# PatrizioPerugini/depth_completion_MT

Hardware: AMD Instinct MI355X
Metric: depth frames/sec at 1216x352 (KITTI); achieved HBM GB/s vs peak (higher is better)
Workload: dtype f32

## Files before the change

### depth_completion_mt_amd/csrc/dcmt.hip

```cpp
#include <hip/hip_runtime.h>

#include <cmath>
#include <cstdio>
#include <cstdlib>
#include <cstdint>
#include <cstring>
#include <algorithm>
#include <new>
#include <type_traits>
#include <vector>

#include "dcmt.h"
#include "dcmt_plan.h"
#include "dcmt_kernels_v1.h"
#include "dcmt_kernels_fused.h"
#include "dcmt_kernels_pair.h"
#include "dcmt_kernels_fp_q16.h"
#include "dcmt_kernels_tail.h"
#include "dcmt_kernels_slic.h"
#include "dcmt_kernels_eval.h"
#include "dcmt_kernels_color.h"
#include "dcmt_cloud.h"

using namespace dcmt;
// ... 47 lines not shown
    uint32_t* cloud_slab = nullptr;
};

namespace {

using plan::TH;
using plan::TW;
using plan::FTH_FEW;

static_assert(plan::kK0AsCompiled == K0_AS_COMPILED && plan::kK0Diamond == K0_DIAMOND, "k0 presets");
static_assert(plan::pre_p_vw(K0_AS_COMPILED, false) == PreP<K0_AS_COMPILED, false>::VW && plan::pre_p_vw(K0_DIAMOND, false) == PreP<K0_DIAMOND, false>::VW &&
              plan::pre_p_vw(K0_AS_COMPILED, true) == PreP<K0_AS_COMPILED, true>::VW && plan::pre_p_vw(K0_DIAMOND, true) == PreP<K0_DIAMOND, true>::VW, "PreP::VW");
static_assert(plan::pre_s_vw(K0_AS_COMPILED, false) == PreS<K0_AS_COMPILED, false>::VW && plan::pre_s_vw(K0_AS_COMPILED, true) == PreS<K0_AS_COMPILED, true>::VW &&
              plan::pre_s_vw(K0_DIAMOND, false) == PreS<K0_DIAMOND, false>::VW && plan::pre_s_vw(K0_DIAMOND, true) == PreS<K0_DIAMOND, true>::VW, "PreS::VW");
static_assert(plan::kFpQVW == FpQ::VW && plan::kPostSVW == PostS::VW && plan::kFillSVW == FillS::VW, "FpQ / PostS / FillS::VW");
static_assert(plan::kMaxBands == kMaxBands && plan::kLabelGroupMax == kLabelGroupMax, "kMaxBands, kLabelGroupMax");
static_assert(plan::kStageNormalize == DCMT_STAGE_NORMALIZE && plan::kStageClose5 == DCMT_STAGE_CLOSE5 && plan::kStageFill7 == DCMT_STAGE_FILL7 &&
              plan::kStageExtend == DCMT_STAGE_EXTEND && plan::kStageFinal == DCMT_STAGE_FINAL, "dcmt_stage");
static_assert(plan::kFlagForceStaged == DCMT_FLAG_FORCE_STAGED && plan::kFlagForceFused == DCMT_FLAG_FORCE_FUSED &&
              plan::kFlagNormalize == DCMT_FLAG_NORMALIZE, "DCMT_FLAG_*");
static_assert(plan::q16_params_ok(100.0f, 0.1f) && Q16::params_ok(100.0f, 0.1f) && !plan::q16_params_ok(80.0f, 0.1f) && !Q16::params_ok(80.0f, 0.1f) &&
              !plan::q16_params_ok(100.0f, 0.2f) && !Q16::params_ok(100.0f, 0.2f), "Q16::params_ok");
static_assert(sizeof(plan::Plan::path) == sizeof(dcmt_ctx::last_path), "dcmt_last_path");

#define DCMT_HIP(ctx, call)                                        \
    do {                                                           \
        hipError_t e_ = (call);                                    \
        if (e_ != hipSuccess) {                                    \
            if (ctx) (ctx)->last_hip_error = (int)e_;              \
            return e_ == hipErrorOutOfMemory ? DCMT_E_NOMEM : DCMT_E_HIP; \
// ... 194 lines not shown
    const float scale = src16 ? fr.in_scale : 1.0f;
    auto pre_s = [&](auto kind, auto wide_) {
        constexpr int KIND = decltype(kind)::value;
        constexpr bool WIDE = decltype(wide_)::value;
        auto* k = d_x4 ? k_pre_s<KIND, WIDE, true, false> : src16 ? k_pre_s<KIND, false, false, true> :
                  cf ? k_pre_s<KIND, WIDE, false, false, true> : k_pre_s<KIND, WIDE, false, false>;
        hipLaunchKernelGGL(k, dim3(pl.pre_grid), b256, 0, st, in, o6, rows, cols, pl.pre_strips, batch, xm, p->max_depth, p->valid_thresh,
                           scale, cf, tc, cnt);
    };
    auto pre_p = [&](auto kind, auto qout, float* o, int* qbad, const int* gate, int* qclr) {
        constexpr int KIND = decltype(kind)::value;
        constexpr bool QOUT = decltype(qout)::value;
        auto* k = d_x4 ? k_pre_p<KIND, true, false, false, QOUT> : src16 ? k_pre_p<KIND, false, true, false, QOUT> :
                  cf ? k_pre_p<KIND, false, false, true> : k_pre_p<KIND, false, false, false, QOUT>;
        hipLaunchKernelGGL(k, dim3(pl.pre_grid), b256, 0, st, in, o, rows, cols, pl.pre_strips, bands, batch, xm, p->max_depth,
                           p->valid_thresh, scale, cf, tc, cnt, qbad, gate, ctx->q16_seen_dev, qclr);
    };
    int* qbad = ctx->q16_bad;
    if (q16) {
        qbad = ctx->q16_bad + ctx->q16_attempts % kQ16Flags;
        int* qnext = ctx->q16_bad + (ctx->q16_attempts + 1) % kQ16Flags;
        ++ctx->q16_attempts;
        with_k0(pl.k0kind, [&](auto kind) { pre_p(kind, std::true_type{}, reinterpret_cast<float*>(ctx->x6q), qbad, nullptr, qnext); });
    } else if (pl.pair) {
        with_k0(pl.k0kind, [&](auto kind) { pre_p(kind, std::false_type{}, o6, nullptr, nullptr, nullptr); });
    } else {
        with_k0(pl.k0kind, [&](auto kind) { if (pl.wide) pre_s(kind, std::true_type{}); else pre_s(kind, std::false_type{}); });
    }
    DCMT_HIP(ctx, hipGetLastError());
    stamp(2);
    if (stop == DCMT_STAGE_EXTEND) {
// ... 2 lines not shown
    }

    const int fstrips = pl.fill_strips, pstrips = pl.post_strips;
    const dim3 fgrid(pl.fill_grid);
    auto fill_apps = [&](int* apps) {
        return fill_loop(ctx, batch, p, st, sync_loop, [&](int i) {
            hipLaunchKernelGGL(k_fill_s, fgrid, b256, 0, st, (i & 1) ? pp0 : pp1, (i & 1) ? pp1 : pp0, cnt, rows, cols,
                               fstrips, batch, xm, p->valid_thresh, i, 0, (const int*)nullptr, 1, (const unsigned short*)nullptr, (const int*)nullptr);
        }, apps);
    };
    if (pl.fuse_fp) {
        const int n_redo = pl.n_redo;
        if (q16) {
            auto* fpq = filled ? k_fp_q<true, true> : bl ? k_fp_q<true, false> : k_fp_q<false, false>;
            hipLaunchKernelGGL(fpq, dim3(pl.fp_q_grid), b256, 0, st, (const void*)ctx->x6q, dst, cnt, rows, cols, pl.q_strips, batch, xm,
                               p->max_depth, p->valid_thresh, (const int*)tc, bands);
            with_k0(pl.k0kind, [&](auto kind) { pre_p(kind, std::false_type{}, x6, nullptr, qbad, nullptr); });
        }
        if (pl.fp_s_launch) {
            auto* fps = filled ? k_fp_s<true, true> : bl ? k_fp_s<true> : k_fp_s<false>;
            hipLaunchKernelGGL(fps, dim3(pl.fp_s_grid), b256, 0, st, x6, dst, cnt, rows, cols, pstrips, batch, xm, p->max_depth,
                               p->valid_thresh, (const int*)tc, bands, q16 ? (const int*)qbad : (const int*)nullptr, pl.fb_s);
        }
        DCMT_HIP(ctx, hipGetLastError());
        stamp(3);
        ctx->last_has_loop = 1;
        int rc = DCMT_OK, apps = 0;
        if (pl.tail) {
            auto* kt = filled ? k_tail<true, true> : bl ? k_tail<true, false> : k_tail<false, false>;
            hipLaunchKernelGGL(kt, dim3(batch), b256, 0, st, (const float*)x6, q16 ? (const unsigned short*)ctx->x6q : (const unsigned short*)nullptr,
                               q16 ? (const int*)qbad : (const int*)nullptr, pp0, pp1, dst, cnt, n_redo, rows, cols, fstrips, pstrips, p->max_depth,
// ... 922 lines not shown
```

### depth_completion_mt_amd/csrc/dcmt_kernels_fp_q16.h

```cpp
#pragma once

#include "dcmt_kernels_pair.h"
#include "median_pk3_nets.h"

namespace dcmt {

typedef unsigned short us2v __attribute__((ext_vector_type(2)));
__device__ __forceinline__ unsigned qmax(unsigned a, unsigned b)
{
    return __builtin_bit_cast(unsigned, __builtin_elementwise_max(__builtin_bit_cast(us2v, a), __builtin_bit_cast(us2v, b)));
}
__device__ __forceinline__ unsigned qmin(unsigned a, unsigned b)
{
    return __builtin_bit_cast(unsigned, __builtin_elementwise_min(__builtin_bit_cast(us2v, a), __builtin_bit_cast(us2v, b)));
}
__device__ __forceinline__ unsigned umax2(unsigned a, unsigned b) { return a > b ? a : b; }

typedef _Float16 hf2v __attribute__((ext_vector_type(2)));
__device__ __forceinline__ unsigned hmax2(unsigned a, unsigned b)
{
    return __builtin_bit_cast(unsigned, __builtin_elementwise_maximum(__builtin_bit_cast(hf2v, a), __builtin_bit_cast(hf2v, b)));
}
__device__ __forceinline__ unsigned hmin2(unsigned a, unsigned b)
{
// ... 107 lines not shown
struct FpQ {
    static constexpr int H = 4;
    static constexpr int VW = 128 - 2 * H;
};

template <bool BLUR>
struct PostPipeP {
    F2 G1[8], MR[8];
    F2 last_out;
    FrameBuf of;
    unsigned ob;
    int rows, cols, gx, rle, rlo;
    bool outlane, edge_strip, outside;
    float max_depth, thr;

    __device__ __forceinline__ void init(float* out_frame, int rows_, int cols_, int gx0, int lane, float max_depth_, float thr_)
    {
        of.init(out_frame, (size_t)rows_ * cols_); rows = rows_; cols = cols_; max_depth = max_depth_; thr = thr_;
        gx = gx0 + 2 * lane;
        ob = 4u * (unsigned)min(max(gx, 0), cols - 2);
        outside = gx < 0 || gx >= cols;
        outlane = !outside && 2 * lane >= FpQ::H && 2 * lane < 128 - FpQ::H;
        rle = (reflect101(gx, cols) - gx0) >> 1;
        rlo = (reflect101(gx + 1, cols) - 1 - gx0) >> 1;
        edge_strip = gx0 < 0 || gx0 + 127 >= cols;
        last_out = {0.f, 0.f};
#pragma unroll
        for (int q = 0; q < 8; ++q) { G1[q] = {0.f, 0.f}; MR[q] = {0.f, 0.f}; }
    }

    enum { BORDER = 0, INNER = 1 };

    template <int PP, int MODE = BORDER>
    __device__ __forceinline__ void after_median(float me, float mo, int u)
    {
        MR[(PP + 4) & 7] = {me, mo};
        if constexpr (BLUR) {
            F2 mf = {me, mo};
            if (edge_strip) {
// ... 68 lines not shown
};

#ifndef DCMT_FPQ_WAVES
#define DCMT_FPQ_WAVES 0
#endif
#ifndef DCMT_FPQ_PFD
#define DCMT_FPQ_PFD 6
#endif
template <bool BLUR, bool FILLED>
__global__ __launch_bounds__(256)
#if DCMT_FPQ_WAVES
__attribute__((amdgpu_waves_per_eu(DCMT_FPQ_WAVES, DCMT_FPQ_WAVES)))
#endif
void k_fp_q(const void* __restrict__ x6_, float* __restrict__ dst, int* __restrict__ counters,
            int rows_all, int cols, int strips, int batch, int xcd_map, float max_depth, float thr, const int* __restrict__ tb,
            int tbands)
{
    __shared__ unsigned s_delay[4][16 * (64 + 64 + 32)];
    const int lane = threadIdx.x & 63;
    const int wave = __builtin_amdgcn_readfirstlane(threadIdx.x >> 6);
    int f, strip;
    if (!wave_strip(blockIdx.x, wave, strips, batch, xcd_map, f, strip)) return;
    int* cnt = frame_counters(counters, f);
    const size_t fo = (size_t)f * rows_all * cols;
    const int gx0 = strip * FpQ::VW - FpQ::H;
    const int gxe = gx0 + 2 * lane;
    const int gxb = lane < 8 ? gx0 + 128 + 2 * lane : (lane < 16 ? gx0 + 128 + 2 * (lane - 8) + 1 :
                    (lane >= 56 ? gx0 - 16 + 2 * (lane - 56) : (lane >= 48 ? gx0 - 16 + 2 * (lane - 48) + 1 : gx0 + 128)));
    const int gxec = min(max(gxe, 0), cols - 2), gxoc = gxec + 1, gxbc = min(max(gxb, 0), cols - 1);
    int tie = 0, tio = 0, tib = 0, bie = rows_all - 1, bio = rows_all - 1, bib = rows_all - 1, V = 0;
    if (tb) {
        table_rows(tb, f, cols, tbands, rows_all, gxec, tie, bie);
        table_rows(tb, f, cols, tbands, rows_all, gxoc, tio, bio);
        table_rows(tb, f, cols, tbands, rows_all, gxbc, tib, bib);
        V = __builtin_amdgcn_readfirstlane(max(wave_min_i(min(min(tie, tio), tib)) - 8, 0));
    }
    const int rows = rows_all - V;
    constexpr unsigned EB = 2;
    FrameBuf sf;
    sf.init(reinterpret_cast<const float*>(static_cast<const char*>(x6_) + fo * EB), (size_t)rows_all * cols * EB / 4);
    const unsigned rowb = EB * (unsigned)cols;
    const unsigned sbe = EB * (unsigned)gxec + (unsigned)V * rowb, sbo = sbe + EB, sbb = EB * (unsigned)gxbc + (unsigned)V * rowb;
    const unsigned fle = EB * (unsigned)gxec + (unsigned)max(tie, V) * rowb, cee = EB * (unsigned)gxec + (unsigned)max(bie, V) * rowb;
    const unsigned flo = EB * (unsigned)gxoc + (unsigned)max(tio, V) * rowb, ceo = EB * (unsigned)gxoc + (unsigned)max(bio, V) * rowb;
    const unsigned flb = EB * (unsigned)gxbc + (unsigned)max(tib, V) * rowb, ceb = EB * (unsigned)gxbc + (unsigned)max(bib, V) * rowb;
    auto clamp3 = [](unsigned a, unsigned lo, unsigned hi) -> unsigned { unsigned r; asm("v_med3_u32 %0, %1, %2, %3" : "=v"(r) : "v"(a), "v"(lo), "v"(hi)); return r; };
    auto ld_code = [&](unsigned off) -> unsigned short { return (unsigned short)__builtin_amdgcn_raw_buffer_load_b16(sf.rs, off, 0, 0); };
    struct Raw { unsigned short e, o, b; };
    auto ld_row = [&](int row) -> Raw {
        return Raw{ld_code(clamp3(sbe + (unsigned)row * rowb, fle, cee)), ld_code(clamp3(sbo + (unsigned)row * rowb, flo, ceo)),
                   ld_code(clamp3(sbb + (unsigned)row * rowb, flb, ceb))};
    };
    auto pack = [](unsigned short e, unsigned short o) -> unsigned { return (unsigned)e | ((unsigned)o << 16); };
    const bool outside = gxe < 0 || gxe >= cols;
    const bool own = !outside && 2 * lane >= FpQ::H && 2 * lane < 128 - FpQ::H;
    const unsigned long long own_mask = __ballot(own);
    const bool edge_strip = gx0 < 0 || gx0 + 127 >= cols;
    const int rep_l = min(max((0 - gx0) >> 1, 0), 63), rep_r = min(max((cols - 2 - gx0) >> 1, 0), 63);
    const int a_m8 = ((lane - 8) & 63) * 4, a_p8 = ((lane + 8) & 63) * 4;
    const bool b_lo = lane < 8, b_hi = lane >= 56;
    unsigned* sd = s_delay[wave];
    unsigned (*dl_c)[64] = reinterpret_cast<unsigned (*)[64]>(sd);
    unsigned (*dl_a)[64] = reinterpret_cast<unsigned (*)[64]>(sd + 16 * 64);
    unsigned (*dl_b)[32] = reinterpret_cast<unsigned (*)[32]>(sd + 16 * 128);
    const int lb = lane < 16 ? lane : (lane >= 48 ? lane - 32 : 0);

    PostPipeP<BLUR> pipe;
    pipe.init(dst + fo + (size_t)V * cols, rows, cols, gx0, lane, max_depth, thr);
    MedianColumnQ mc;
    mc.init();

    const bool warm = V > 0;
    unsigned xa0 = 0, xb0 = 0;
    if (warm) { const Raw r = ld_row(0); xa0 = pack(r.e, r.o); xb0 = r.b; }
    unsigned short PFE[16], PFO[16], PFB[16];
    unsigned PFA[16], W2A[16], W6A[16], W2B[16], W6B[16];
#pragma unroll
    for (int q = 0; q < 16; ++q) { PFE[q] = PFO[q] = PFB[q] = 0; PFA[q] = 0; W2A[q] = W6A[q] = xa0; W2B[q] = W6B[q] = xb0; }
#pragma unroll
    for (int q = 0; q < 16; ++q) { dl_c[q][lane] = xa0; dl_a[q][lane] = xa0; dl_b[q][lb] = xb0; }
    constexpr int PFD = DCMT_FPQ_PFD;
#pragma unroll
    for (int q = 0; q < PFD; ++q) {
        const Raw r = ld_row(min(max(q + (warm ? 16 : 0) - 15, 0), rows - 1));
        PFE[q] = r.e; PFO[q] = r.o; PFB[q] = r.b;
    }
    unsigned vpa = xa0, vpb = xb0, x7_prev = xa0;
    int before = 0, after = 0;
    unsigned pend_v = xa0, pend_f1 = 0, pend_f2 = 0;
    unsigned long long pend_hme = 0, pend_hmo = 0;
    unsigned nxt_c = xa0, nxt_a = xa0, nxt_b = xb0;

    using Pipe = PostPipeP<BLUR>;
    using BorderMode = std::integral_constant<int, Pipe::BORDER>;
    auto fill_step = [&](auto P_, auto M_, int t) -> unsigned {
        constexpr int p = decltype(P_)::value;
        constexpr int MODE = decltype(M_)::value;
        unsigned xa;
        const unsigned xb = PFB[p];
        if constexpr (MODE == Pipe::BORDER) {
            xa = pack(PFE[p], PFO[p]);
            const Raw r = ld_row(min(max(t + PFD - 15, 0), rows - 1));
            PFE[(p + PFD) & 15] = r.e; PFO[(p + PFD) & 15] = r.o; PFB[(p + PFD) & 15] = r.b;
        } else {
            xa = PFA[p];
            const unsigned srow = (unsigned)(t + PFD - 15) * rowb;
            PFA[(p + PFD) & 15] = (unsigned)__builtin_amdgcn_raw_buffer_load_b32(sf.rs, sbe, srow, 0);
            PFB[(p + PFD) & 15] = (unsigned short)__builtin_amdgcn_raw_buffer_load_b16(sf.rs, sbb, srow, 0);
        }
        const int o = t - 31;
        unsigned x7 = pend_v;
        if ((pend_hme | pend_hmo) != 0ull) {
            const unsigned d = qmax(pend_f1, pend_f2);
            const bool he = __builtin_amdgcn_inverse_ballot_w64(pend_hme), ho = __builtin_amdgcn_inverse_ballot_w64(pend_hmo);
            const unsigned m = (he ? 0xffffu : 0u) | (ho ? 0xffff0000u : 0u);
            x7 = (d & m) | (pend_v & ~m);
            if (MODE != Pipe::BORDER || (unsigned)o < (unsigned)rows) {
                before += __builtin_popcountll(pend_hme & own_mask) + __builtin_popcountll(pend_hmo & own_mask);
                after += __builtin_popcountll(__builtin_amdgcn_ballot_w64((x7 << 16) <= Q16::HOLE_MAX_HI) & own_mask) +
                         __builtin_popcountll(__builtin_amdgcn_ballot_w64(x7 <= Q16::HOLE_MAX_HI) & own_mask);
            }
        }
        if (edge_strip) {
            const unsigned l0 = (unsigned)__shfl((int)x7, rep_l, 64), r0 = (unsigned)__shfl((int)x7, rep_r, 64);
            if (gxe < 0) x7 = (l0 & 0xffffu) | (l0 << 16);
            if (gxe >= cols) x7 = (r0 >> 16) | (r0 & 0xffff0000u);
        }
        if (MODE == Pipe::BORDER && o >= rows) { asm volatile("" ::); x7 = x7_prev; }
        x7_prev = x7;
        const unsigned w2a = hmax2(xa, vpa);
        vpa = xa;
        W2A[p] = w2a;
        const unsigned w6a = hmax3(w2a, W2A[(p + 14) & 15], W2A[(p + 12) & 15]);
        W6A[p] = w6a;
        const unsigned w18a = hmax3(w6a, W6A[(p + 10) & 15], W6A[(p + 4) & 15]);
// ... 51 lines not shown
                    post_step(std::integral_constant<int, 2>{}, BorderMode{}, x7, 2);
                }
            }
        });
    }
    const int nsteps = rows + 35;
    int t0 = 32;
    auto main_step = [&](auto P_) {
        constexpr int p = decltype(P_)::value;
        const int t = t0 + p, u = t - 29;
        const unsigned x7 = fill_step(P_, BorderMode{}, t);
        post_step(std::integral_constant<int, ((p + 3) & 7)>{}, BorderMode{}, x7, u);
        if constexpr (p == 3) {
            if (t0 == 32 && V > 0) {
                FrameBuf top;
                top.init(dst + fo, (size_t)V * cols);
                const unsigned tbo = pipe.outlane ? pipe.ob : kDropOffset;
                for (int r = 0; r < V; ++r) st2(top, tbo, r, cols, pipe.last_out);
            }
        }
    };
    const int r_first = max(__builtin_amdgcn_readfirstlane(wave_max_i(max(max(tie, tio), tib))) - V, 0);
    const int r_last = min(__builtin_amdgcn_readfirstlane(wave_min_i(min(min(bie, bio), bib))) - V, rows - 1);
    auto interior = [&](int t) -> bool { return t >= 48 && t + PFD - 15 >= r_first && t + PFD <= r_last; };
    using InnerMode = std::integral_constant<int, Pipe::INNER>;
    for (; t0 < nsteps; t0 += 16) {
        if (interior(t0)) {
#pragma unroll
            for (int q = 0; q < PFD; ++q) PFA[q] = pack(PFE[q], PFO[q]);
            do {
                static_for<0, 16>([&](auto P_) {
// ... 4 lines not shown
                    post_step(std::integral_constant<int, ((p + 3) & 7)>{}, InnerMode{}, x7, t - 29);
                });
                t0 += 16;
            } while (interior(t0));
#pragma unroll
            for (int q = 0; q < PFD; ++q) { PFE[q] = (unsigned short)PFA[q]; PFO[q] = (unsigned short)(PFA[q] >> 16); }
        }
        static_for<0, 4>(main_step);
        if (t0 + 4 >= nsteps) break;
        static_for<4, 8>(main_step);
        if (t0 + 8 >= nsteps) break;
        static_for<8, 12>(main_step);
        if (t0 + 12 >= nsteps) break;
        static_for<12, 16>(main_step);
    }
    if (lane == 0) {
        if (before) atomicAdd(&cnt[0], before);
        if (after) atomicAdd(&cnt[1], after);
    }
}

}
```

### depth_completion_mt_amd/csrc/dcmt_kernels_fused.h

```cpp
#pragma once

#include <type_traits>

#include "dcmt_kernels_v1.h"

namespace dcmt {

__device__ __forceinline__ float from_left(float v)
{
    return __builtin_bit_cast(float, __builtin_amdgcn_update_dpp(0, __builtin_bit_cast(int, v), 0x138 , 0xf, 0xf, true));
}
__device__ __forceinline__ float from_right(float v)
{
    return __builtin_bit_cast(float, __builtin_amdgcn_update_dpp(0, __builtin_bit_cast(int, v), 0x130 , 0xf, 0xf, true));
}

__device__ __forceinline__ float hmax3(float v) { const float a = fmax2(from_left(v), v); return fmax2(from_right(a), a); }
__device__ __forceinline__ float hmin3(float v) { const float a = fmin2(from_left(v), v); return fmin2(from_right(a), a); }
__device__ __forceinline__ float hgrow_max(float w) { const float l = from_left(w); return fmax2(from_right(w), l); }
__device__ __forceinline__ float hgrow_min(float w) { const float l = from_left(w); return fmin2(from_right(w), l); }

constexpr unsigned kDropOffset = 0x7ffffff0u;
struct FrameBuf {
    __amdgpu_buffer_rsrc_t rs;
// ... 59 lines not shown
}

__device__ __forceinline__ bool wave_strip(int b, int wave, int strips, int batch, int xcd_map, int& f, int& strip)
{
    if (xcd_map) {
        const int g = (b >> 3) * 4 + wave;
        if (g >= (batch >> 3) * strips) return false;
        f = (g / strips) * 8 + (b & 7);
        strip = g % strips;
    } else {
        const int g = b * 4 + wave;
        if (g >= batch * strips) return false;
        f = g / strips;
        strip = g % strips;
    }
    return true;
}

__device__ __forceinline__ void clear_frame_counters(int* counters, int f, bool first_wave_of_frame, int lane)
{
    if (counters && first_wave_of_frame)
        for (int i = lane; i < kCntStride; i += 64) counters[(size_t)f * kCntStride + i] = 0;
}

__device__ __forceinline__ void table_rows(const int* tb, int f, int cols, int bands, int rows, int c, int& first, int& last)
{
    const int* tt = tb + (size_t)f * bands * 2 * cols + c;
    first = tt[0]; last = tt[cols];
    if (bands > 1) {
        for (int b = 1; b < bands; ++b) { first = min(first, tt[(size_t)b * 2 * cols]); last = max(last, tt[(size_t)b * 2 * cols + cols]); }
// ... 844 lines not shown
```

### depth_completion_mt_amd/csrc/dcmt_kernels_pair.h

```cpp
#pragma once

#include "dcmt_kernels_fused.h"

namespace dcmt {

struct F2 { float e, o; };

__device__ __forceinline__ F2 p_max(F2 a, F2 b) { return {fmax2(a.e, b.e), fmax2(a.o, b.o)}; }
__device__ __forceinline__ F2 p_max3(F2 a, F2 b, F2 c) { return {fmax3(a.e, b.e, c.e), fmax3(a.o, b.o, c.o)}; }
__device__ __forceinline__ F2 p_min3(F2 a, F2 b, F2 c) { return {fmin3(a.e, b.e, c.e), fmin3(a.o, b.o, c.o)}; }
__device__ __forceinline__ F2 p_sel(bool c, F2 a, F2 b) { return {c ? a.e : b.e, c ? a.o : b.o}; }
__device__ __forceinline__ F2 p_hmax3(F2 v) { const float m = fmax2(v.e, v.o); return {fmax2(from_left(v.o), m), fmax2(from_right(v.e), m)}; }
__device__ __forceinline__ F2 p_hmin3(F2 v) { const float m = fmin2(v.e, v.o); return {fmin2(from_left(v.o), m), fmin2(from_right(v.e), m)}; }
__device__ __forceinline__ F2 p_grow_max(F2 w) { return {fmax2(from_left(w.o), w.o), fmax2(from_right(w.e), w.e)}; }
__device__ __forceinline__ F2 p_grow_min(F2 w) { return {fmin2(from_left(w.o), w.o), fmin2(from_right(w.e), w.e)}; }

typedef unsigned u2v __attribute__((ext_vector_type(2)));
typedef float f2v __attribute__((ext_vector_type(2)));
__device__ __forceinline__ F2 ld2(const FrameBuf& b, unsigned lane_bytes, int row, int cols)
{
    const f2v v = __builtin_bit_cast(f2v, __builtin_amdgcn_raw_buffer_load_b64(b.rs, lane_bytes, row * cols * 4, 0));
    return {v.x, v.y};
}
__device__ __forceinline__ void st2(const FrameBuf& b, unsigned lane_bytes, int row, int cols, F2 v)
{
    const f2v f = {v.e, v.o};
    __builtin_amdgcn_raw_buffer_store_b64(__builtin_bit_cast(u2v, f), b.rs, lane_bytes, row * cols * 4, 0);
}

template <int K0KIND, bool START4>
struct PreP {
    static constexpr int HL0 = START4 ? 3 : (K0KIND == K0_AS_COMPILED ? 0 : 2) + 2 + 2 + 3;
    static constexpr int HR0 = START4 ? 3 : 2 + 2 + 2 + 3;
    static constexpr int HL = (HL0 + 3) / 4 * 4;
    static constexpr int VW = (128 - HL - HR0) / 4 * 4;
    static constexpr int LAT = 9;
};

constexpr int kMaxBands = 8;


#ifndef DCMT_PRE_WAVES
#define DCMT_PRE_WAVES 0
#endif
template <int K0KIND, bool START4 = false, bool U16 = false, bool NORM = false, bool Q16OUT = false>
__global__ __launch_bounds__(256)
#if DCMT_PRE_WAVES
__attribute__((amdgpu_waves_per_eu(DCMT_PRE_WAVES, DCMT_PRE_WAVES)))
#endif
void k_pre_p(const void* __restrict__ src_, float* __restrict__ x6, int rows, int cols, int strips, int bands,
             int batch, int xcd_map, float max_depth, float thr, float in_scale, const float* __restrict__ coef,
             int* __restrict__ tb, int* __restrict__ counters, int* __restrict__ q16_bad, const int* __restrict__ gate, int* __restrict__ q16_seen,
             int* __restrict__ q16_clear)
{
    static_assert(!(U16 && START4), "the uint16 ingest is the first kernel of the path");
    static_assert(!(NORM && (U16 || START4)), "normalisation applies to raw f32 frames");
    static_assert(!(NORM && Q16OUT), "normalised frames are not multiples of 1/256");
    if (gate && *gate == 0) return;
    if (q16_clear && blockIdx.x == 0 && threadIdx.x == 0) *q16_clear = 0;
    const float* src = static_cast<const float*>(src_);
    using G = PreP<K0KIND, START4>;
    constexpr int ROFF = START4 ? 6 : 0;
    const int lane = threadIdx.x & 63;
    const int wave = __builtin_amdgcn_readfirstlane(threadIdx.x >> 6);
    int f, unit;
    if (!wave_strip(blockIdx.x, wave, strips * bands, batch, xcd_map, f, unit)) return;
    const int strip = unit / bands, band = unit - strip * bands;
    clear_frame_counters(counters, f, unit == 0, lane);
    const int gx0 = strip * G::VW - G::HL;
    const int gx = gx0 + 2 * lane;
    const bool incol = gx >= 0 && gx < cols;
    const bool outlane = incol && 2 * lane >= G::HL && 2 * lane < G::HL + G::VW;
    const size_t fo = (size_t)f * rows * cols;
    const int gxc = min(max(gx, 0), cols - 2);
    float na = 1.0f, nb = 0.0f;
    if constexpr (NORM) { na = coef[2 * f]; nb = coef[2 * f + 1]; }
    FrameBuf ob, ib;
    if constexpr (Q16OUT) ob.init(reinterpret_cast<const float*>(reinterpret_cast<const unsigned short*>(x6) + fo), (size_t)rows * cols / 2);
    else ob.init(x6 + fo, (size_t)rows * cols);
    if constexpr (U16) ib.init(reinterpret_cast<const float*>(static_cast<const uint16_t*>(src_) + fo), (size_t)rows * cols / 2);
    else ib.init(src + fo, (size_t)rows * cols);
    const unsigned oc = 4u * (unsigned)gxc;
    const unsigned qc = 2u * (unsigned)gxc;
    unsigned bad = 0;
    auto load_row = [&](int r) -> F2 {
        if constexpr (U16) {
            const unsigned w = __builtin_amdgcn_raw_buffer_load_b32(ib.rs, 2u * (unsigned)gxc, r * cols * 2, 0);
            return {__fmul_rn((float)(w & 0xffffu), in_scale), __fmul_rn((float)(w >> 16), in_scale)};
        } else {
            return ld2(ib, oc, r, cols);
        }
    };

    const int r0 = (int)((long long)rows * band / bands), r1 = (int)((long long)rows * (band + 1) / bands);

    constexpr float NEG = -FLT_MAX, POS = FLT_MAX;
    const F2 NEG2 = {NEG, NEG}, POS2 = {POS, POS};
    F2 PF[8];
// ... 149 lines not shown
        } else {
            st2(ob, sa, inrows ? m : 0, cols, x5);
        }
    };
    const bool strip_inner = gx0 >= 0 && gx0 + 127 < cols;
    const int inner_lo = max(START4 ? 6 + ROFF : 6, m0 + 9), inner_hi = min(rows + ROFF - PFD, r1 + 9);
    int i0 = S;
    for (; i0 < nsteps && !(strip_inner && i0 >= inner_lo && i0 + 7 < inner_hi); i0 += 8)
        static_for<0, 8>([&](auto P_) { row_step(std::false_type{}, P_, i0 + decltype(P_)::value); });
    for (; i0 < nsteps && strip_inner && i0 + 7 < inner_hi; i0 += 8)
        static_for<0, 8>([&](auto P_) { row_step(std::true_type{}, P_, i0 + decltype(P_)::value); });
    for (; i0 < nsteps; i0 += 8)
        static_for<0, 8>([&](auto P_) { row_step(std::false_type{}, P_, i0 + decltype(P_)::value); });
    if constexpr (Q16OUT && !START4 && !U16) bad |= (chk_max > 35838u ? 1u : 0u) | chk_or;
    if (tb) {
        int* tt = tb + ((size_t)f * bands + band) * 2 * cols, *bt = tt + cols;
        if (outlane) {
            const bool ee = bie < 0, eo = bio < 0;
            if ((ee | eo) && band == bands - 1) {
                asm volatile("s_waitcnt vmcnt(0)" ::: "memory");
                if constexpr (Q16OUT) {
                    if (ee) __builtin_amdgcn_raw_buffer_store_b16((short)Q16::CODE_MAX, ob.rs, qc + 2u * (unsigned)((rows - 1) * cols), 0, 0);
                    if (eo) __builtin_amdgcn_raw_buffer_store_b16((short)Q16::CODE_MAX, ob.rs, qc + 2u + 2u * (unsigned)((rows - 1) * cols), 0, 0);
                } else {
                    if (ee) ob.st_at(oc + 4u * (unsigned)((rows - 1) * cols), 100.0f);
                    if (eo) ob.st_at(oc + 4u + 4u * (unsigned)((rows - 1) * cols), 100.0f);
                }
            }
            const bool tr = bands == 1;
            *reinterpret_cast<int2*>(tt + gx) = make_int2(ee && tr ? rows - 1 : tie, eo && tr ? rows - 1 : tio);
            *reinterpret_cast<int2*>(bt + gx) = make_int2(ee && tr ? rows - 1 : bie, eo && tr ? rows - 1 : bio);
// ... 202 lines not shown
```

### depth_completion_mt_amd/csrc/dcmt_plan.h

```cpp
#ifndef DCMT_PLAN_H
#define DCMT_PLAN_H

#include <cmath>
#include <cstddef>
#include <cstdint>
#include <cstdlib>

namespace dcmt {
namespace plan {

struct Knobs {
    int poison = 0;
    int xcd_map = 1;
    int wide = 1;
    int fuse_fp = 1;
    int top_table = 1;
    int pair = 1;
    int bands = 0;
    int fbands = 0;
    int fp_q16 = 1;
    int assume_filled = 1;
    int q16_min_waves = 2600;
    int bbox_global = 0;
    int label_group = 0;
    int label_pairs = -1;
    int min_fused_batch = 3;
};

struct KnobEnv { const char* name; int Knobs::* member; char parse; };
constexpr KnobEnv kKnobEnv[] = {
    {"DCMT_POISON", &Knobs::poison, '1'},
    {"DCMT_XCD_MAP", &Knobs::xcd_map, 'i'},
    {"DCMT_WIDE", &Knobs::wide, 'i'},
    {"DCMT_FUSE_FP", &Knobs::fuse_fp, 'i'},
    {"DCMT_TOP_TABLE", &Knobs::top_table, 'i'},
    {"DCMT_PAIR", &Knobs::pair, 'i'},
    {"DCMT_BANDS", &Knobs::bands, 'i'},
    {"DCMT_FBANDS", &Knobs::fbands, 'i'},
    {"DCMT_FP_Q16", &Knobs::fp_q16, 'i'},
    {"DCMT_ASSUME_FILLED", &Knobs::assume_filled, 'i'},
    {"DCMT_Q16_MIN_WAVES", &Knobs::q16_min_waves, 'i'},
    {"DCMT_BBOX_GLOBAL", &Knobs::bbox_global, 'p'},
    {"DCMT_LABEL_GROUP", &Knobs::label_group, 'i'},
    {"DCMT_LABEL_PAIRS", &Knobs::label_pairs, 'i'},
    {"DCMT_MIN_FUSED_BATCH", &Knobs::min_fused_batch, 'i'},
};

inline Knobs knobs_from_env()
{
    Knobs k;
    for (const KnobEnv& e : kKnobEnv) {
        const char* v = std::getenv(e.name);
        if (v) k.*e.member = e.parse == 'i' ? std::atoi(v) : e.parse == '1' ? v[0] == '1' : 1;
    }
    return k;
}

constexpr int TH = 32, TW = 64;
constexpr int FTH_FEW = 16;
constexpr int kFewFrames = 12;
constexpr int kK0AsCompiled = 0, kK0Diamond = 1;
constexpr int pre_p_vw(int k0kind, bool start4) { return start4 ? 120 : k0kind == kK0AsCompiled ? 108 : 104; }
constexpr int pre_s_vw(int k0kind, bool wide) { return k0kind == kK0AsCompiled ? (wide ? 44 : 48) : (wide ? 40 : 46); }
constexpr int kFpQVW = 120, kPostSVW = 56, kFillSVW = 34;
constexpr int kMaxBands = 8;
constexpr int kLabelGroupMax = 4;
constexpr int kPreBandWaves = 2560;
constexpr int kFpSOneBandWaves = 2048, kFpSBandWaves = 3072;
constexpr bool q16_params_ok(float max_depth, float thr) { return max_depth == 100.0f && thr == 0.1f; }
constexpr int kStageNormalize = 1, kStageClose5 = 4, kStageFill7 = 5, kStageExtend = 6, kStageFinal = 11;
constexpr int kFlagForceStaged = 1, kFlagForceFused = 2, kFlagNormalize = 4;
constexpr const char* kPathCopy = " + copy to dst";

enum class Input { F32, U16, LABELED };

struct Call {
    int rows = 0, cols = 0, batch = 0;
    Input input = Input::F32;
    int n_labels = 0;
// ... 18 lines not shown
    Out out = Out::DST;
    bool needs_x6q = false, needs_colstat = false, needs_bbox = false;
    bool few = false;
    int tile_h = TH, tiles_x = 0, tiles_y = 0;
    bool u16_convert = false;
    int dump = 0;
    bool bbox_lds = false, lpair = false, label_pairs = false;
    int label_group = 1, label_grid_x = 0;
    bool table = false;
    bool wide = false, pair = false, q16 = false;
    int bands = 1, fb_s = 1;
    int pre_strips = 0, fill_strips = 0, post_strips = 0, q_strips = 0;
    unsigned pre_grid = 0, fill_grid = 0, post_grid = 0, fp_s_grid = 0, fp_q_grid = 0;
    bool fuse_fp = false;
    bool filled = false, tail = false, fp_s_launch = false;
    int n_redo = 0;
    char path[160] = "";
};

inline bool ranges_overlap(uintptr_t a, size_t a_bytes, uintptr_t b, size_t b_bytes) { return a < b + b_bytes && b < a + a_bytes; }

inline unsigned wave_grid(int strips, int batch, int xcd_map)
{
    return xcd_map ? 8 * (((batch / 8) * strips + 3) / 4) : (batch * strips + 3) / 4;
}

inline void path_append(char (&path)[160], const char* s)
{
    size_t n = 0;
    while (path[n]) ++n;
    while (*s && n + 1 < sizeof path) path[n++] = *s++;
    path[n] = 0;
}

inline Route route_of(const Knobs& k, const Call& c)
{
    if ((c.flags & kFlagNormalize) && c.stop_after == kStageNormalize) return Route::NORMALIZE_ONLY;
    const bool big_enough = c.batch >= k.min_fused_batch || (c.flags & kFlagForceFused);
    const bool streaming = !(c.flags & kFlagForceStaged) && big_enough && c.k0kind >= 0 && c.rows >= 8 && c.cols >= 8;
// ... 58 lines not shown
        p.wide = k.wide && cols % 4 == 0 && src % 16 == 0 && !u16;
        p.pair = k.pair && cols % 2 == 0 && cols >= 8 && src % (u16 ? 4 : 8) == 0 && o6 % 8 == 0;
        if (p.pair && p.table) {
            const long long w1 = (long long)batch * ((cols + pre_p_vw(kK0AsCompiled, false) - 1) / pre_p_vw(kK0AsCompiled, false));
            p.bands = k.bands > 0 ? k.bands : (w1 >= kPreBandWaves ? 1 : (int)((kPreBandWaves + w1 - 1) / w1));
            if (p.bands > rows / 32) p.bands = rows / 32 > 0 ? rows / 32 : 1;
            if (p.bands > kMaxBands) p.bands = kMaxBands;
        }
        p.q_strips = (cols + kFpQVW - 1) / kFpQVW;
        p.q16 = k.fp_q16 && c.q16_allowed && (long long)batch * p.q_strips >= k.q16_min_waves && p.pair && p.table && !cf &&
                q16_params_ok(c.max_depth, c.valid_thresh) && c.dst % 8 == 0 && (!u16 || c.in_scale == 0.00390625f) && !overlap;
        p.needs_x6q = p.q16;
        const int vw = p.pair ? pre_p_vw(c.k0kind, labeled) : pre_s_vw(c.k0kind, p.wide);
        p.pre_strips = (cols + vw - 1) / vw;
        p.pre_grid = wave_grid(p.pre_strips * p.bands, batch, p.xcd_map);
        if (labeled) path_append(p.path, "k_label_bbox + k_label_stage + ");
        path_append(p.path, p.q16 ? (u16 ? "k_pre_p<U16,Q16OUT>" : "k_pre_p<Q16OUT>") :
                            p.pair ? (labeled ? "k_pre_p<START4>" : u16 ? "k_pre_p<U16>" : cf ? "k_pre_p<NORM>" : "k_pre_p") : "k_pre_s");
        if (p.bands > 1) path_append(p.path, " (row bands)");
        if (stop == kStageExtend) {
            if (p.out != Out::DST) path_append(p.path, kPathCopy);
            return p;
        }
        p.fill_strips = (cols + kFillSVW - 1) / kFillSVW;
        p.fill_grid = (unsigned)((p.fill_strips + 3) / 4) * batch;
        p.post_strips = (cols + kPostSVW - 1) / kPostSVW;
        p.post_grid = (unsigned)((p.post_strips + 3) / 4) * batch;
        if (!p.fuse_fp) return p;
        if (p.table) {
            const long long w1 = (long long)batch * p.post_strips;
            p.fb_s = k.fbands > 0 ? k.fbands : (w1 >= kFpSOneBandWaves ? 1 : (int)((kFpSBandWaves + w1 / 2) / w1));
            if (p.fb_s > rows / 32) p.fb_s = rows / 32 > 0 ? rows / 32 : 1;
            if (p.fb_s < 1) p.fb_s = 1;
        }
        p.filled = c.gaussian && k.assume_filled && (c.sync_loop || (c.spec_fill_iters >= 1 && c.max_fill_iters >= 1));
        p.n_redo = c.sync_loop ? c.max_fill_iters : (c.spec_fill_iters < c.max_fill_iters ? c.spec_fill_iters : c.max_fill_iters);
        p.tail = !c.sync_loop && p.n_redo > 0;
        p.fp_s_launch = !p.q16 || !p.tail;
        p.fp_q_grid = wave_grid(p.q_strips, batch, p.xcd_map);
        p.fp_s_grid = wave_grid(p.post_strips * p.fb_s, batch, p.xcd_map);
        path_append(p.path, p.q16 ? " + k_fp_q" : (p.fb_s > 1 ? " + k_fp_s (row bands)" : " + k_fp_s"));
        return p;
    }

    p.needs_colstat = true;
    p.few = batch < kFewFrames;
    p.tile_h = p.few ? FTH_FEW : TH;
    p.tiles_x = (cols + TW - 1) / TW;
    p.tiles_y = (rows + p.tile_h - 1) / p.tile_h;
    p.u16_convert = u16;
    if (u16) overlap = false;
    p.dump = stop <= kStageClose5 ? stop : 0;
    p.out = stop <= kStageFill7 && overlap ? (stop == kStageFill7 ? Out::X5 : Out::PP0) : Out::DST;
    path_append(p.path, labeled ? "k_pre_labeled_v1" : "k_pre_v1");
// ... 10 lines not shown
```

Before: 742,000.

## Pack last-strip remainders of two frames into one wave in pre_p and fp_q

For the rightmost column strip, which covers only a narrow remainder of each frame, one wave now handles the remainders of two frames, using its two 32-lane halves with a frame-offset buffer resource. Odd-group frames skip their last strip, and hole counters are accumulated and flushed separately per half. The goal is to cut the number of mostly idle edge waves in the Q16 pre and fused fill/post kernels. It also sets a waves-per-EU occupancy hint on the Q16 pre kernel. The cost is more complex indexing, extra ballots and popcounts, and buffer-range assumptions guarded by plan checks.

```diff
diff --git a/depth_completion_mt_amd/csrc/dcmt.hip b/depth_completion_mt_amd/csrc/dcmt.hip
--- a/depth_completion_mt_amd/csrc/dcmt.hip
+++ b/depth_completion_mt_amd/csrc/dcmt.hip
@@ -85,6 +85,11 @@
 static_assert(plan::pre_s_vw(K0_AS_COMPILED, false) == PreS<K0_AS_COMPILED, false>::VW && plan::pre_s_vw(K0_AS_COMPILED, true) == PreS<K0_AS_COMPILED, true>::VW &&
               plan::pre_s_vw(K0_DIAMOND, false) == PreS<K0_DIAMOND, false>::VW && plan::pre_s_vw(K0_DIAMOND, true) == PreS<K0_DIAMOND, true>::VW, "PreS::VW");
 static_assert(plan::kFpQVW == FpQ::VW && plan::kPostSVW == PostS::VW && plan::kFillSVW == FillS::VW, "FpQ / PostS / FillS::VW");
+static_assert(plan::pre_p_hl(K0_AS_COMPILED) == PreP<K0_AS_COMPILED, false>::HL && plan::pre_p_hl(K0_DIAMOND) == PreP<K0_DIAMOND, false>::HL &&
+              plan::kPrePHR0 == PreP<K0_AS_COMPILED, false>::HR0 && plan::kPrePHR0 == PreP<K0_DIAMOND, false>::HR0 &&
+              PreP<K0_AS_COMPILED, false>::HALF_IN == plan::kHalfWaveCols - (plan::kPrePHR0 + 1) / 2 * 2, "k_pre_p's remainder strips in pairs");
+static_assert(plan::kFpQH == FpQ::H && plan::kHalfWaveCols == 64 && plan::kFillReach == 15 && plan::kPairSpanBytesMax < kDropOffset,
+              "k_fp_q's remainder strips in pairs: FpQ::H, the half-wave, the reach of the 31-wide maximum, one buffer resource for both frames");
 static_assert(plan::kMaxBands == kMaxBands && plan::kLabelGroupMax == kLabelGroupMax, "kMaxBands, kLabelGroupMax");
 static_assert(plan::kStageNormalize == DCMT_STAGE_NORMALIZE && plan::kStageClose5 == DCMT_STAGE_CLOSE5 && plan::kStageFill7 == DCMT_STAGE_FILL7 &&
               plan::kStageExtend == DCMT_STAGE_EXTEND && plan::kStageFinal == DCMT_STAGE_FINAL, "dcmt_stage");
@@ -309,7 +314,7 @@
         auto* k = d_x4 ? k_pre_p<KIND, true, false, false, QOUT> : src16 ? k_pre_p<KIND, false, true, false, QOUT> :
                   cf ? k_pre_p<KIND, false, false, true> : k_pre_p<KIND, false, false, false, QOUT>;
         hipLaunchKernelGGL(k, dim3(pl.pre_grid), b256, 0, st, in, o, rows, cols, pl.pre_strips, bands, batch, xm, p->max_depth,
-                           p->valid_thresh, scale, cf, tc, cnt, qbad, gate, ctx->q16_seen_dev, qclr);
+                           p->valid_thresh, scale, cf, tc, cnt, qbad, gate, ctx->q16_seen_dev, qclr, QOUT && pl.pre_edge_pairs ? 1 : 0);
     };
     int* qbad = ctx->q16_bad;
     if (q16) {
@@ -342,7 +347,7 @@
         if (q16) {
             auto* fpq = filled ? k_fp_q<true, true> : bl ? k_fp_q<true, false> : k_fp_q<false, false>;
             hipLaunchKernelGGL(fpq, dim3(pl.fp_q_grid), b256, 0, st, (const void*)ctx->x6q, dst, cnt, rows, cols, pl.q_strips, batch, xm,
-                               p->max_depth, p->valid_thresh, (const int*)tc, bands);
+                               p->max_depth, p->valid_thresh, (const int*)tc, bands, pl.fp_q_edge_pairs ? 1 : 0);
             with_k0(pl.k0kind, [&](auto kind) { pre_p(kind, std::false_type{}, x6, nullptr, qbad, nullptr); });
         }
         if (pl.fp_s_launch) {
diff --git a/depth_completion_mt_amd/csrc/dcmt_kernels_fp_q16.h b/depth_completion_mt_amd/csrc/dcmt_kernels_fp_q16.h
--- a/depth_completion_mt_amd/csrc/dcmt_kernels_fp_q16.h
+++ b/depth_completion_mt_amd/csrc/dcmt_kernels_fp_q16.h
@@ -145,15 +145,16 @@
     bool outlane, edge_strip, outside;
     float max_depth, thr;
 
-    __device__ __forceinline__ void init(float* out_frame, int rows_, int cols_, int gx0, int lane, float max_depth_, float thr_)
+    __device__ __forceinline__ void init(float* out_frame, int rows_, int cols_, int gx0, int ll, int lane0, unsigned fpx, unsigned span, bool own,
+                                         float max_depth_, float thr_)
     {
-        of.init(out_frame, (size_t)rows_ * cols_); rows = rows_; cols = cols_; max_depth = max_depth_; thr = thr_;
-        gx = gx0 + 2 * lane;
-        ob = 4u * (unsigned)min(max(gx, 0), cols - 2);
+        of.init(out_frame, (size_t)span + (size_t)rows_ * cols_); rows = rows_; cols = cols_; max_depth = max_depth_; thr = thr_;
+        gx = gx0 + 2 * ll;
+        ob = 4u * ((unsigned)min(max(gx, 0), cols - 2) + fpx);
         outside = gx < 0 || gx >= cols;
-        outlane = !outside && 2 * lane >= FpQ::H && 2 * lane < 128 - FpQ::H;
-        rle = (reflect101(gx, cols) - gx0) >> 1;
-        rlo = (reflect101(gx + 1, cols) - 1 - gx0) >> 1;
+        outlane = own;
+        rle = lane0 + ((reflect101(gx, cols) - gx0) >> 1);
+        rlo = lane0 + ((reflect101(gx + 1, cols) - 1 - gx0) >> 1);
         edge_strip = gx0 < 0 || gx0 + 127 >= cols;
         last_out = {0.f, 0.f};
 #pragma unroll
@@ -252,36 +253,45 @@
 #endif
 void k_fp_q(const void* __restrict__ x6_, float* __restrict__ dst, int* __restrict__ counters,
             int rows_all, int cols, int strips, int batch, int xcd_map, float max_depth, float thr, const int* __restrict__ tb,
-            int tbands)
+            int tbands, int edge_pairs)
 {
     __shared__ unsigned s_delay[4][16 * (64 + 64 + 32)];
     const int lane = threadIdx.x & 63;
     const int wave = __builtin_amdgcn_readfirstlane(threadIdx.x >> 6);
     int f, strip;
     if (!wave_strip(blockIdx.x, wave, strips, batch, xcd_map, f, strip)) return;
-    int* cnt = frame_counters(counters, f);
+    int fd = 0;
+    if (edge_pairs && strip == strips - 1 && !edge_pair_partner(f, batch, xcd_map, fd)) return;
+    const bool paired = fd != 0;
+    const int lane0 = paired ? lane & 32 : 0, ll = lane - lane0;
+    const int fl = lane0 ? f + fd : f;
+    const unsigned span = (unsigned)fd * (unsigned)(rows_all * cols);
+    const unsigned fpx = lane0 ? span : 0u;
     const size_t fo = (size_t)f * rows_all * cols;
-    const int gx0 = strip * FpQ::VW - FpQ::H;
-    const int gxe = gx0 + 2 * lane;
+    const int own0 = strip * FpQ::VW;
+    const int gx0 = paired ? cols - (64 - FpQ::H) : own0 - FpQ::H;
+    const int gxe = gx0 + 2 * ll;
     const int gxb = lane < 8 ? gx0 + 128 + 2 * lane : (lane < 16 ? gx0 + 128 + 2 * (lane - 8) + 1 :
                     (lane >= 56 ? gx0 - 16 + 2 * (lane - 56) : (lane >= 48 ? gx0 - 16 + 2 * (lane - 48) + 1 : gx0 + 128)));
     const int gxec = min(max(gxe, 0), cols - 2), gxoc = gxec + 1, gxbc = min(max(gxb, 0), cols - 1);
     int tie = 0, tio = 0, tib = 0, bie = rows_all - 1, bio = rows_all - 1, bib = rows_all - 1, V = 0;
     if (tb) {
-        table_rows(tb, f, cols, tbands, rows_all, gxec, tie, bie);
-        table_rows(tb, f, cols, tbands, rows_all, gxoc, tio, bio);
-        table_rows(tb, f, cols, tbands, rows_all, gxbc, tib, bib);
+        table_rows(tb, fl, cols, tbands, rows_all, gxec, tie, bie);
+        table_rows(tb, fl, cols, tbands, rows_all, gxoc, tio, bio);
+        table_rows(tb, fl, cols, tbands, rows_all, paired ? gxec : gxbc, tib, bib);
         V = __builtin_amdgcn_readfirstlane(max(wave_min_i(min(min(tie, tio), tib)) - 8, 0));
     }
     const int rows = rows_all - V;
     constexpr unsigned EB = 2;
     FrameBuf sf;
-    sf.init(reinterpret_cast<const float*>(static_cast<const char*>(x6_) + fo * EB), (size_t)rows_all * cols * EB / 4);
+    sf.init(reinterpret_cast<const float*>(static_cast<const char*>(x6_) + fo * EB), ((size_t)span + (size_t)rows_all * cols) * EB / 4);
     const unsigned rowb = EB * (unsigned)cols;
-    const unsigned sbe = EB * (unsigned)gxec + (unsigned)V * rowb, sbo = sbe + EB, sbb = EB * (unsigned)gxbc + (unsigned)V * rowb;
-    const unsigned fle = EB * (unsigned)gxec + (unsigned)max(tie, V) * rowb, cee = EB * (unsigned)gxec + (unsigned)max(bie, V) * rowb;
-    const unsigned flo = EB * (unsigned)gxoc + (unsigned)max(tio, V) * rowb, ceo = EB * (unsigned)gxoc + (unsigned)max(bio, V) * rowb;
-    const unsigned flb = EB * (unsigned)gxbc + (unsigned)max(tib, V) * rowb, ceb = EB * (unsigned)gxbc + (unsigned)max(bib, V) * rowb;
+    const unsigned cbe = EB * ((unsigned)gxec + fpx), cbo = cbe + EB;
+    const unsigned cbb = paired ? kDropOffset : EB * (unsigned)gxbc, vb = paired ? 0u : (unsigned)V;
+    const unsigned sbe = cbe + (unsigned)V * rowb, sbo = sbe + EB, sbb = cbb + vb * rowb;
+    const unsigned fle = cbe + (unsigned)max(tie, V) * rowb, cee = cbe + (unsigned)max(bie, V) * rowb;
+    const unsigned flo = cbo + (unsigned)max(tio, V) * rowb, ceo = cbo + (unsigned)max(bio, V) * rowb;
+    const unsigned flb = paired ? kDropOffset : cbb + (unsigned)max(tib, V) * rowb, ceb = paired ? kDropOffset : cbb + (unsigned)max(bib, V) * rowb;
     auto clamp3 = [](unsigned a, unsigned lo, unsigned hi) -> unsigned { unsigned r; asm("v_med3_u32 %0, %1, %2, %3" : "=v"(r) : "v"(a), "v"(lo), "v"(hi)); return r; };
     auto ld_code = [&](unsigned off) -> unsigned short { return (unsigned short)__builtin_amdgcn_raw_buffer_load_b16(sf.rs, off, 0, 0); };
     struct Raw { unsigned short e, o, b; };
@@ -291,11 +301,11 @@
     };
     auto pack = [](unsigned short e, unsigned short o) -> unsigned { return (unsigned)e | ((unsigned)o << 16); };
     const bool outside = gxe < 0 || gxe >= cols;
-    const bool own = !outside && 2 * lane >= FpQ::H && 2 * lane < 128 - FpQ::H;
-    const unsigned long long own_mask = __ballot(own);
+    const bool own = !outside && gxe >= own0 && gxe < own0 + FpQ::VW;
+    const unsigned long long own_all = __ballot(own), own_mask = paired ? own_all & 0xffffffffull : own_all, own_mask2 = own_all & ~own_mask;
     const bool edge_strip = gx0 < 0 || gx0 + 127 >= cols;
-    const int rep_l = min(max((0 - gx0) >> 1, 0), 63), rep_r = min(max((cols - 2 - gx0) >> 1, 0), 63);
-    const int a_m8 = ((lane - 8) & 63) * 4, a_p8 = ((lane + 8) & 63) * 4;
+    const int rep_l = min(max((0 - gx0) >> 1, 0), 63), rep_r = lane0 + min(max((cols - 2 - gx0) >> 1, 0), 63);
+    const int a_m8 = ((lane - 8) & 63) * 4, a_p8 = (paired && (lane >> 3) == 3 ? lane - 24 : (lane + 8) & 63) * 4;
     const bool b_lo = lane < 8, b_hi = lane >= 56;
     unsigned* sd = s_delay[wave];
     unsigned (*dl_c)[64] = reinterpret_cast<unsigned (*)[64]>(sd);
@@ -304,7 +314,7 @@
     const int lb = lane < 16 ? lane : (lane >= 48 ? lane - 32 : 0);
 
     PostPipeP<BLUR> pipe;
-    pipe.init(dst + fo + (size_t)V * cols, rows, cols, gx0, lane, max_depth, thr);
+    pipe.init(dst + fo + (size_t)V * cols, rows, cols, gx0, ll, lane0, fpx, span, own, max_depth, thr);
     MedianColumnQ mc;
     mc.init();
 
@@ -324,7 +334,7 @@
         PFE[q] = r.e; PFO[q] = r.o; PFB[q] = r.b;
     }
     unsigned vpa = xa0, vpb = xb0, x7_prev = xa0;
-    int before = 0, after = 0;
+    int before = 0, after = 0, before2 = 0, after2 = 0;
     unsigned pend_v = xa0, pend_f1 = 0, pend_f2 = 0;
     unsigned long long pend_hme = 0, pend_hmo = 0;
     unsigned nxt_c = xa0, nxt_a = xa0, nxt_b = xb0;
@@ -354,9 +364,11 @@
             const unsigned m = (he ? 0xffffu : 0u) | (ho ? 0xffff0000u : 0u);
             x7 = (d & m) | (pend_v & ~m);
             if (MODE != Pipe::BORDER || (unsigned)o < (unsigned)rows) {
+                const unsigned long long ae = __builtin_amdgcn_ballot_w64((x7 << 16) <= Q16::HOLE_MAX_HI), ao = __builtin_amdgcn_ballot_w64(x7 <= Q16::HOLE_MAX_HI);
                 before += __builtin_popcountll(pend_hme & own_mask) + __builtin_popcountll(pend_hmo & own_mask);
-                after += __builtin_popcountll(__builtin_amdgcn_ballot_w64((x7 << 16) <= Q16::HOLE_MAX_HI) & own_mask) +
-                         __builtin_popcountll(__builtin_amdgcn_ballot_w64(x7 <= Q16::HOLE_MAX_HI) & own_mask);
+                after += __builtin_popcountll(ae & own_mask) + __builtin_popcountll(ao & own_mask);
+                before2 += __builtin_popcountll(pend_hme & own_mask2) + __builtin_popcountll(pend_hmo & own_mask2);
+                after2 += __builtin_popcountll(ae & own_mask2) + __builtin_popcountll(ao & own_mask2);
             }
         }
         if (edge_strip) {
@@ -438,7 +450,7 @@
         if constexpr (p == 3) {
             if (t0 == 32 && V > 0) {
                 FrameBuf top;
-                top.init(dst + fo, (size_t)V * cols);
+                top.init(dst + fo, (size_t)span + (size_t)V * cols);
                 const unsigned tbo = pipe.outlane ? pipe.ob : kDropOffset;
                 for (int r = 0; r < V; ++r) st2(top, tbo, r, cols, pipe.last_out);
             }
@@ -473,10 +485,12 @@
         if (t0 + 12 >= nsteps) break;
         static_for<12, 16>(main_step);
     }
-    if (lane == 0) {
-        if (before) atomicAdd(&cnt[0], before);
-        if (after) atomicAdd(&cnt[1], after);
-    }
-}
-
-}
+    if (lane == 0 || (paired && lane == 32)) {
+        int* cnt = frame_counters(counters, fl);
+        const int b = lane0 ? before2 : before, a = lane0 ? after2 : after;
+        if (b) atomicAdd(&cnt[0], b);
+        if (a) atomicAdd(&cnt[1], a);
+    }
+}
+
+}
diff --git a/depth_completion_mt_amd/csrc/dcmt_kernels_fused.h b/depth_completion_mt_amd/csrc/dcmt_kernels_fused.h
--- a/depth_completion_mt_amd/csrc/dcmt_kernels_fused.h
+++ b/depth_completion_mt_amd/csrc/dcmt_kernels_fused.h
@@ -97,6 +97,15 @@
         f = g / strips;
         strip = g % strips;
     }
+    return true;
+}
+
+__device__ __forceinline__ bool edge_pair_partner(int f, int batch, int xcd_map, int& fd)
+{
+    const int grp = xcd_map ? f >> 3 : f, ngrp = xcd_map ? batch >> 3 : batch;
+    fd = 0;
+    if (grp & 1) return false;
+    if (grp + 1 < ngrp) fd = xcd_map ? 8 : 1;
     return true;
 }
 
diff --git a/depth_completion_mt_amd/csrc/dcmt_kernels_pair.h b/depth_completion_mt_amd/csrc/dcmt_kernels_pair.h
--- a/depth_completion_mt_amd/csrc/dcmt_kernels_pair.h
+++ b/depth_completion_mt_amd/csrc/dcmt_kernels_pair.h
@@ -35,6 +35,7 @@
     static constexpr int HL = (HL0 + 3) / 4 * 4;
     static constexpr int VW = (128 - HL - HR0) / 4 * 4;
     static constexpr int LAT = 9;
+    static constexpr int HALF_IN = 64 - (HR0 + 1) / 2 * 2;
 };
 
 constexpr int kMaxBands = 8;
@@ -47,11 +48,13 @@
 __global__ __launch_bounds__(256)
 #if DCMT_PRE_WAVES
 __attribute__((amdgpu_waves_per_eu(DCMT_PRE_WAVES, DCMT_PRE_WAVES)))
+#else
+__attribute__((amdgpu_waves_per_eu(Q16OUT && !START4 && !U16 ? (K0KIND == K0_AS_COMPILED ? 5 : 4) : 1)))
 #endif
 void k_pre_p(const void* __restrict__ src_, float* __restrict__ x6, int rows, int cols, int strips, int bands,
              int batch, int xcd_map, float max_depth, float thr, float in_scale, const float* __restrict__ coef,
              int* __restrict__ tb, int* __restrict__ counters, int* __restrict__ q16_bad, const int* __restrict__ gate, int* __restrict__ q16_seen,
-             int* __restrict__ q16_clear)
+             int* __restrict__ q16_clear, int edge_pairs)
 {
     static_assert(!(U16 && START4), "the uint16 ingest is the first kernel of the path");
     static_assert(!(NORM && (U16 || START4)), "normalisation applies to raw f32 frames");
@@ -67,21 +70,32 @@
     if (!wave_strip(blockIdx.x, wave, strips * bands, batch, xcd_map, f, unit)) return;
     const int strip = unit / bands, band = unit - strip * bands;
     clear_frame_counters(counters, f, unit == 0, lane);
-    const int gx0 = strip * G::VW - G::HL;
-    const int gx = gx0 + 2 * lane;
+    constexpr bool PAIRABLE = Q16OUT && !START4 && !U16;
+    int fd = 0;
+    if constexpr (PAIRABLE) {
+        if (edge_pairs && strip == strips - 1 && !edge_pair_partner(f, batch, xcd_map, fd)) return;
+    }
+    const bool paired = fd != 0;
+    const int lane0 = paired ? lane & 32 : 0, ll = lane - lane0;
+    const int fl = lane0 ? f + fd : f;
+    const unsigned span = (unsigned)fd * (unsigned)(rows * cols);
+    const unsigned fpx = lane0 ? span : 0u;
+    const int own0 = strip * G::VW;
+    const int gx0 = paired ? cols - G::HALF_IN : own0 - G::HL;
+    const int gx = gx0 + 2 * ll;
     const bool incol = gx >= 0 && gx < cols;
-    const bool outlane = incol && 2 * lane >= G::HL && 2 * lane < G::HL + G::VW;
+    const bool outlane = incol && gx >= own0 && gx < own0 + G::VW;
     const size_t fo = (size_t)f * rows * cols;
     const int gxc = min(max(gx, 0), cols - 2);
     float na = 1.0f, nb = 0.0f;
     if constexpr (NORM) { na = coef[2 * f]; nb = coef[2 * f + 1]; }
     FrameBuf ob, ib;
-    if constexpr (Q16OUT) ob.init(reinterpret_cast<const float*>(reinterpret_cast<const unsigned short*>(x6) + fo), (size_t)rows * cols / 2);
+    if constexpr (Q16OUT) ob.init(reinterpret_cast<const float*>(reinterpret_cast<const unsigned short*>(x6) + fo), ((size_t)span + (size_t)rows * cols) / 2);
     else ob.init(x6 + fo, (size_t)rows * cols);
     if constexpr (U16) ib.init(reinterpret_cast<const float*>(static_cast<const uint16_t*>(src_) + fo), (size_t)rows * cols / 2);
-    else ib.init(src + fo, (size_t)rows * cols);
-    const unsigned oc = 4u * (unsigned)gxc;
-    const unsigned qc = 2u * (unsigned)gxc;
+    else ib.init(src + fo, (size_t)span + (size_t)rows * cols);
+    const unsigned oc = 4u * ((unsigned)gxc + fpx);
+    const unsigned qc = 2u * ((unsigned)gxc + fpx);
     unsigned bad = 0;
     auto load_row = [&](int r) -> F2 {
         if constexpr (U16) {
@@ -261,7 +275,7 @@
         static_for<0, 8>([&](auto P_) { row_step(std::false_type{}, P_, i0 + decltype(P_)::value); });
     if constexpr (Q16OUT && !START4 && !U16) bad |= (chk_max > 35838u ? 1u : 0u) | chk_or;
     if (tb) {
-        int* tt = tb + ((size_t)f * bands + band) * 2 * cols, *bt = tt + cols;
+        int* tt = tb + ((size_t)fl * bands + band) * 2 * cols, *bt = tt + cols;
         if (outlane) {
             const bool ee = bie < 0, eo = bio < 0;
             if ((ee | eo) && band == bands - 1) {
diff --git a/depth_completion_mt_amd/csrc/dcmt_plan.h b/depth_completion_mt_amd/csrc/dcmt_plan.h
--- a/depth_completion_mt_amd/csrc/dcmt_plan.h
+++ b/depth_completion_mt_amd/csrc/dcmt_plan.h
@@ -24,6 +24,7 @@
     int bbox_global = 0;
     int label_group = 0;
     int label_pairs = -1;
+    int edge_pairs = 1;
     int min_fused_batch = 3;
 };
 
@@ -43,6 +44,7 @@
     {"DCMT_BBOX_GLOBAL", &Knobs::bbox_global, 'p'},
     {"DCMT_LABEL_GROUP", &Knobs::label_group, 'i'},
     {"DCMT_LABEL_PAIRS", &Knobs::label_pairs, 'i'},
+    {"DCMT_EDGE_PAIRS", &Knobs::edge_pairs, 'i'},
     {"DCMT_MIN_FUSED_BATCH", &Knobs::min_fused_batch, 'i'},
 };
 
@@ -63,6 +65,11 @@
 constexpr int pre_p_vw(int k0kind, bool start4) { return start4 ? 120 : k0kind == kK0AsCompiled ? 108 : 104; }
 constexpr int pre_s_vw(int k0kind, bool wide) { return k0kind == kK0AsCompiled ? (wide ? 44 : 48) : (wide ? 40 : 46); }
 constexpr int kFpQVW = 120, kPostSVW = 56, kFillSVW = 34;
+constexpr int pre_p_hl(int k0kind) { return k0kind == kK0AsCompiled ? 8 : 12; }
+constexpr int kPrePHR0 = 9;
+constexpr int kFpQH = 4, kFillReach = 15, kHalfWaveCols = 64;
+constexpr int kPairSpanFrames = 9;
+constexpr unsigned long long kPairSpanBytesMax = 0x7fffffc0ull;
 constexpr int kMaxBands = 8;
 constexpr int kLabelGroupMax = 4;
 constexpr int kPreBandWaves = 2560;
@@ -111,6 +118,7 @@
     unsigned pre_grid = 0, fill_grid = 0, post_grid = 0, fp_s_grid = 0, fp_q_grid = 0;
     bool fuse_fp = false;
     bool filled = false, tail = false, fp_s_launch = false;
+    bool pre_edge_pairs = false, fp_q_edge_pairs = false;
     int n_redo = 0;
     char path[160] = "";
 };
@@ -120,6 +128,22 @@
 inline unsigned wave_grid(int strips, int batch, int xcd_map)
 {
     return xcd_map ? 8 * (((batch / 8) * strips + 3) / 4) : (batch * strips + 3) / 4;
+}
+
+inline bool fp_q_pairs(int rows, int cols, int q_strips, int xcd_map)
+{
+    if (q_strips < 2 || cols % 2 != 0) return false;
+    const int R = cols - kFpQVW * (q_strips - 1);
+    if (R + kFpQH + kFillReach + kFpQH > kHalfWaveCols) return false;
+    return (unsigned long long)(xcd_map ? kPairSpanFrames : 2) * rows * cols * 4 <= kPairSpanBytesMax;
+}
+
+inline bool pre_p_pairs(int rows, int cols, int k0kind, int pre_strips, int bands, int xcd_map)
+{
+    if (bands != 1 || pre_strips < 2 || cols % 2 != 0) return false;
+    const int R = cols - pre_p_vw(k0kind, false) * (pre_strips - 1);
+    if (R + pre_p_hl(k0kind) + (kPrePHR0 + 1) / 2 * 2 > kHalfWaveCols) return false;
+    return (unsigned long long)(xcd_map ? kPairSpanFrames : 2) * rows * cols * 4 <= kPairSpanBytesMax;
 }
 
 inline void path_append(char (&path)[160], const char* s)
@@ -208,6 +232,7 @@
         const int vw = p.pair ? pre_p_vw(c.k0kind, labeled) : pre_s_vw(c.k0kind, p.wide);
         p.pre_strips = (cols + vw - 1) / vw;
         p.pre_grid = wave_grid(p.pre_strips * p.bands, batch, p.xcd_map);
+        p.pre_edge_pairs = p.q16 && !u16 && !labeled && k.edge_pairs && pre_p_pairs(rows, cols, c.k0kind, p.pre_strips, p.bands, p.xcd_map);
         if (labeled) path_append(p.path, "k_label_bbox + k_label_stage + ");
         path_append(p.path, p.q16 ? (u16 ? "k_pre_p<U16,Q16OUT>" : "k_pre_p<Q16OUT>") :
                             p.pair ? (labeled ? "k_pre_p<START4>" : u16 ? "k_pre_p<U16>" : cf ? "k_pre_p<NORM>" : "k_pre_p") : "k_pre_s");
@@ -232,6 +257,7 @@
         p.tail = !c.sync_loop && p.n_redo > 0;
         p.fp_s_launch = !p.q16 || !p.tail;
         p.fp_q_grid = wave_grid(p.q_strips, batch, p.xcd_map);
+        p.fp_q_edge_pairs = p.q16 && k.edge_pairs && fp_q_pairs(rows, cols, p.q_strips, p.xcd_map);
         p.fp_s_grid = wave_grid(p.post_strips * p.fb_s, batch, p.xcd_map);
         path_append(p.path, p.q16 ? " + k_fp_q" : (p.fb_s > 1 ? " + k_fp_s (row bands)" : " + k_fp_s"));
         return p;
```

Result: slower. 712,400 (-4.0%).
